# MingXiangL/SPE

Hardware: AMD Instinct MI355X
Metric: images/sec (whole node) at 3x800x1333 bs=2/GPU (higher is better)
Workload: dtype bf16/fp16 operands, fp32 accumulate; 1 GPU; TSCAM_cait_S24 (C=384, depth 24, 8 heads) + 0-layer encoder + 6-layer conditional-DETR decoder x2 stages, 100 queries, COCO heads (91), 2x3x800x1333 per GPU (N=4150 tokens), fwd + SetCriterion + SetCriterionRefine + bwd + grad all-reduce + clip + AdamW; global_batch=2, parallelism=dp1

## Files before the change

### spe_amd/csrc/gemm_bf16tn.hip

```cpp
#include "common.h"

#define GT_BR 64

typedef unsigned int u32x4t_t __attribute__((ext_vector_type(4)));
typedef short s16x4t_t __attribute__((ext_vector_type(4)));
typedef short s16x8t_t __attribute__((ext_vector_type(8)));

struct GemmTNArgs {
    const unsigned short* A; const unsigned short* B; float* C;
    int M, N, R; long lda, ldb, ldc; float alpha;
    int splitk; long slab; int rt_per_split;
};

template <int W>
__device__ __forceinline__ void gt_load(const unsigned short* __restrict__ base, long ld, int r0, int R, int c0, int C, u32x4t_t (&v)[W / 32]) {
    constexpr int CPR = W / 8, RPP = 256 / CPR;
    const int t = threadIdx.x, cc = c0 + (t % CPR) * 8;
    const bool cv = cc < C;
    const int ccl = cv ? cc : 0;
#pragma unroll
    for (int i = 0; i < W / 32; ++i) {
        const int r = r0 + t / CPR + RPP * i;
        const bool ok = cv && r < R;
        const u32x4t_t q = *reinterpret_cast<const u32x4t_t*>(base + (long)min(r, R - 1) * ld + ccl);
        v[i] = ok ? q : (u32x4t_t){0u, 0u, 0u, 0u};
    }
}
template <int W>
__device__ __forceinline__ void gt_stage(unsigned short* lds, const u32x4t_t (&v)[W / 32]) {
    constexpr int CPR = W / 8, RPP = 256 / CPR, LD = W + 8;
    const int t = threadIdx.x;
#pragma unroll
    for (int i = 0; i < W / 32; ++i)
        *reinterpret_cast<u32x4t_t*>(lds + (t / CPR + RPP * i) * LD + (t % CPR) * 8) = v[i];
}
template <int LD>
__device__ __forceinline__ bf16x8_t gt_operand(const unsigned short* tile, int ks, int c0, int lane) {
    typedef __attribute__((address_space(3))) s16x4t_t lds_s4;
    const unsigned short* p = tile + (32 * ks + 8 * (lane >> 4) + ((lane & 15) >> 2)) * LD + c0 + 4 * (lane & 3);
    const s16x4t_t v0 = __builtin_amdgcn_ds_read_tr16_b64_v4i16((lds_s4*)(p));
    const s16x4t_t v1 = __builtin_amdgcn_ds_read_tr16_b64_v4i16((lds_s4*)(p + 4 * LD));
    const s16x8t_t v = __builtin_shufflevector(v0, v1, 0, 1, 2, 3, 4, 5, 6, 7);
    return __builtin_bit_cast(bf16x8_t, v);
}

template <int BM, int BN>
__global__ __launch_bounds__(256) void gemm_bf16tn_kernel(GemmTNArgs p) {
    extern __shared__ __attribute__((aligned(16))) unsigned short smem_tn[];
    constexpr int NFM = BM / 32, NFN = BN / 32, WM = BM / 2, WN = BN / 2;
    constexpr int LDA = BM + 8, LDB = BN + 8;
    constexpr int TA_ = GT_BR * LDA, TB_ = GT_BR * LDB;
    auto sA = [&](int buf) { return smem_tn + buf * (TA_ + TB_); };
    auto sB = [&](int buf) { return smem_tn + buf * (TA_ + TB_) + TA_; };
    const int tiles_m = (p.M + BM - 1) / BM;
    const int tm = blockIdx.x % tiles_m, tn = blockIdx.x / tiles_m;
    const int zs = blockIdx.z;
    float* C = p.C + (long)zs * p.slab;
    const int m0 = tm * BM, n0 = tn * BN;
    const int rtiles = (p.R + GT_BR - 1) / GT_BR;
    const int rt_begin = zs * p.rt_per_split;
    int rt_end = rt_begin + p.rt_per_split; if (rt_end > rtiles) rt_end = rtiles;
    const int nt = rt_end - rt_begin;
    const int lane = threadIdx.x & 63, w = threadIdx.x >> 6;
    const int wm = w >> 1, wn = w & 1, fr = lane & 15;

    f32x4_t acc[NFM][NFN];
#pragma unroll
    for (int i = 0; i < NFM; ++i)
#pragma unroll
        for (int j = 0; j < NFN; ++j) acc[i][j] = (f32x4_t){0.f, 0.f, 0.f, 0.f};

    u32x4t_t ca[BM / 32], cb[BN / 32], na[BM / 32], nb[BN / 32];
#pragma unroll
    for (int i = 0; i < BM / 32; ++i) na[i] = (u32x4t_t){0u, 0u, 0u, 0u};
#pragma unroll
    for (int i = 0; i < BN / 32; ++i) nb[i] = (u32x4t_t){0u, 0u, 0u, 0u};
    if (nt > 0) {
        gt_load<BM>(p.A, p.lda, rt_begin * GT_BR, p.R, m0, p.M, ca);
        gt_load<BN>(p.B, p.ldb, rt_begin * GT_BR, p.R, n0, p.N, cb);
        gt_stage<BM>(sA(0), ca);
        gt_stage<BN>(sB(0), cb);
        if (nt > 1) {
            gt_load<BM>(p.A, p.lda, (rt_begin + 1) * GT_BR, p.R, m0, p.M, ca);
            gt_load<BN>(p.B, p.ldb, (rt_begin + 1) * GT_BR, p.R, n0, p.N, cb);
        }
        __syncthreads();
        for (int t = 0; t < nt; ++t) {
            const int buf = t & 1;
            if (t + 2 < nt) {
                gt_load<BM>(p.A, p.lda, (rt_begin + t + 2) * GT_BR, p.R, m0, p.M, na);
                gt_load<BN>(p.B, p.ldb, (rt_begin + t + 2) * GT_BR, p.R, n0, p.N, nb);
            }
#pragma unroll
            for (int ks = 0; ks < GT_BR / 32; ++ks) {
                bf16x8_t a[NFM], b[NFN];
#pragma unroll
                for (int i = 0; i < NFM; ++i) a[i] = gt_operand<LDA>(sA(buf), ks, wm * WM + i * 16, lane);
#pragma unroll
                for (int j = 0; j < NFN; ++j) b[j] = gt_operand<LDB>(sB(buf), ks, wn * WN + j * 16, lane);
#pragma unroll
                for (int i = 0; i < NFM; ++i)
#pragma unroll
                    for (int j = 0; j < NFN; ++j)
                        acc[i][j] = __builtin_amdgcn_mfma_f32_16x16x32_bf16(b[j], a[i], acc[i][j], 0, 0, 0);
            }
            if (t + 1 < nt) {
                gt_stage<BM>(sA(buf ^ 1), ca);
                gt_stage<BN>(sB(buf ^ 1), cb);
            }
#pragma unroll
            for (int i = 0; i < BM / 32; ++i) ca[i] = na[i];
#pragma unroll
            for (int i = 0; i < BN / 32; ++i) cb[i] = nb[i];
            __syncthreads();
        }
    }
    const bool vst = ((p.ldc & 3) == 0) && ((reinterpret_cast<uintptr_t>(C) & 15) == 0);
#pragma unroll
    for (int j = 0; j < NFN; ++j) {
        const int n = n0 + wn * WN + j * 16 + (lane >> 4) * 4;
        if (n >= p.N) continue;
#pragma unroll
        for (int i = 0; i < NFM; ++i) {
            const int m = m0 + wm * WM + i * 16 + fr;
            if (m >= p.M) continue;
            const long off = (long)m * p.ldc + n;
            float v[4];
#pragma unroll
            for (int r = 0; r < 4; ++r) v[r] = acc[i][j][r] * p.alpha;
            if (vst && n + 3 < p.N) spe_store4_stream(C + off, v[0], v[1], v[2], v[3]);
            else {
#pragma unroll
                for (int r = 0; r < 4; ++r) if (n + r < p.N) C[off + r] = v[r];
            }
        }
    }
}

template <int BM, int BN>
static int launch_tn(const GemmTNArgs& p, hipStream_t stream) {
    constexpr int smem = 2 * GT_BR * ((BM + 8) + (BN + 8)) * (int)sizeof(unsigned short);
    static bool attr_set = false;
    if (!attr_set) {
        hipError_t e = hipFuncSetAttribute(reinterpret_cast<const void*>(&gemm_bf16tn_kernel<BM, BN>),
                                           hipFuncAttributeMaxDynamicSharedMemorySize, smem);
        if (e != hipSuccess) return (int)e;
        attr_set = true;
    }
    const int tiles = ((p.M + BM - 1) / BM) * ((p.N + BN - 1) / BN);
    hipLaunchKernelGGL((gemm_bf16tn_kernel<BM, BN>), dim3(tiles, 1, p.splitk), dim3(256), smem, stream, p);
    SPE_CHECK_LAUNCH();
    return 0;
}

struct TnPlan { int BM, BN, splits, rt_per_split; };
static int tn_gemm_select(int M, int N, int R, long lda, long ldb, int splitk, TnPlan* s) {
    if (M <= 0 || N <= 0) return 1;
    if (R <= 0) return -4;
    if ((lda & 7) || (ldb & 7) || (M & 7) || (N & 7)) return -2;
    const int rtiles = (R + GT_BR - 1) / GT_BR;
    if (splitk < 0) { splitk = -splitk; if (splitk > rtiles) return -5; }
    else if (splitk > 1) return -2;
    if (splitk < 1) splitk = 1;
    s->splits = splitk;
    s->rt_per_split = (rtiles + splitk - 1) / splitk;
    const long t128 = (long)((M + 127) / 128) * ((N + 127) / 128) * splitk;
    static const int small_max = SPE_KNOB("SPE_TN_SMALL_TILES", 256);
    if (t128 < small_max) { s->BM = 64; s->BN = 64; }
    else if (M > 64 && N > 64) { s->BM = 128; s->BN = 128; }
    else if (M > 64) { s->BM = 128; s->BN = 64; }
    else { s->BM = 64; s->BN = 64; }
    return 0;
}

extern "C" int spe_gemm_bf16tn_plan(int M, int N, int R, long lda, long ldb, int splitk, int* v) {
    TnPlan s;
    const int rc = tn_gemm_select(M, N, R, lda, ldb, splitk, &s);
    if (rc < 0) return rc;
    if (rc > 0) s = TnPlan{0, 0, 0, 0};
    if (v) { v[0] = s.BM; v[1] = s.BN; v[2] = s.splits; v[3] = s.rt_per_split; }
    return 0;
}

extern "C" int spe_gemm_bf16tn(const void* A16, const void* B16, float* C, int M, int N, int R, long lda, long ldb, long ldc,
                               float alpha, int splitk, hipStream_t stream) {
    TnPlan s;
    const int rc = tn_gemm_select(M, N, R, lda, ldb, splitk, &s);
    if (rc > 0) return 0;
    if (rc == -4) return rc;
    auto al16 = [](const void* q) { return (reinterpret_cast<uintptr_t>(q) & 15) == 0; };
    if (!al16(A16) || !al16(B16)) return -2;
    if (rc < 0) return rc;
    GemmTNArgs p;
    p.A = reinterpret_cast<const unsigned short*>(A16); p.B = reinterpret_cast<const unsigned short*>(B16); p.C = C;
    p.M = M; p.N = N; p.R = R; p.lda = lda; p.ldb = ldb; p.ldc = ldc; p.alpha = alpha;
    p.slab = splitk < 0 ? (long)M * ldc : 0;
    p.splitk = s.splits;
    p.rt_per_split = s.rt_per_split;
    if (s.BM == 64 && s.BN == 64) return launch_tn<64, 64>(p, stream);
    if (s.BM == 128 && s.BN == 128) return launch_tn<128, 128>(p, stream);
    if (s.BM == 128 && s.BN == 64) return launch_tn<128, 64>(p, stream);
    return -2;
}
```

### spe_amd/csrc/gemm_tiles.h

```cpp
#pragma once

struct TileOrder {
    int xcd_bind;
    int grid;
};

static inline TileOrder tile_order(int M, int N, int tiles_m, int tiles_n) {
    TileOrder o{0, tiles_m * tiles_n};
    if (M >= N && tiles_m >= 16) o.xcd_bind = 1;
    else if (N > M && tiles_n >= 16) o.xcd_bind = 2;
    else if (tiles_m >= 16) o.xcd_bind = 1;
    else if (tiles_n >= 16) o.xcd_bind = 2;
    if (o.xcd_bind == 1) o.grid = 8 * ((tiles_m + 7) / 8) * tiles_n;
    if (o.xcd_bind == 2) o.grid = 8 * ((tiles_n + 7) / 8) * tiles_m;
    return o;
}

__device__ __forceinline__ bool tile_decode(int xcd_bind, int tiles_m, int tiles_n, int& tm, int& tn) {
    if (xcd_bind == 0) { tm = blockIdx.x % tiles_m; tn = blockIdx.x / tiles_m; }
    else {
        const int no = (xcd_bind == 1) ? tiles_n : tiles_m;
        const int xcd = blockIdx.x & 7, idx = blockIdx.x >> 3;
        const int tb = xcd + 8 * (idx / no), to = idx % no;
        tm = (xcd_bind == 1) ? tb : to; tn = (xcd_bind == 1) ? to : tb;
        if (tm >= tiles_m || tn >= tiles_n) return false;
    }
    return true;
}

__device__ __forceinline__ void glds16(const void* gsrc, unsigned lds_dst) {
    unsigned keep;
    asm volatile("s_mov_b32 %0, m0\n\ts_mov_b32 m0, %2\n\ts_nop 0\n\tglobal_load_lds_dwordx4 %1, off\n\ts_mov_b32 m0, %0"
                 : "=&s"(keep) : "v"(gsrc), "s"(lds_dst) : "memory");
}
```

Baseline: 41.84 images/sec.

## Remap TN GEMM blocks to XCD-contiguous chunks and unroll 64x64 double-buffer ping-pong

```diff
diff --git a/spe_amd/csrc/gemm_bf16tn.hip b/spe_amd/csrc/gemm_bf16tn.hip
--- a/spe_amd/csrc/gemm_bf16tn.hip
+++ b/spe_amd/csrc/gemm_bf16tn.hip
@@ -1,4 +1,5 @@
 #include "common.h"
+#include "gemm_tiles.h"
 
 #define GT_BR 64
 
@@ -16,23 +17,23 @@
 __device__ __forceinline__ void gt_load(const unsigned short* __restrict__ base, long ld, int r0, int R, int c0, int C, u32x4t_t (&v)[W / 32]) {
     constexpr int CPR = W / 8, RPP = 256 / CPR;
     const int t = threadIdx.x, cc = c0 + (t % CPR) * 8;
-    const bool cv = cc < C;
-    const int ccl = cv ? cc : 0;
+    const int ccl = cc < C ? cc : 0;
 #pragma unroll
     for (int i = 0; i < W / 32; ++i) {
         const int r = r0 + t / CPR + RPP * i;
-        const bool ok = cv && r < R;
-        const u32x4t_t q = *reinterpret_cast<const u32x4t_t*>(base + (long)min(r, R - 1) * ld + ccl);
-        v[i] = ok ? q : (u32x4t_t){0u, 0u, 0u, 0u};
+        v[i] = *reinterpret_cast<const u32x4t_t*>(base + (long)min(r, R - 1) * ld + ccl);
     }
 }
 template <int W>
-__device__ __forceinline__ void gt_stage(unsigned short* lds, const u32x4t_t (&v)[W / 32]) {
+__device__ __forceinline__ void gt_stage(unsigned short* lds, const u32x4t_t (&v)[W / 32], int r0, int R, int c0, int C) {
     constexpr int CPR = W / 8, RPP = 256 / CPR, LD = W + 8;
     const int t = threadIdx.x;
-#pragma unroll
-    for (int i = 0; i < W / 32; ++i)
-        *reinterpret_cast<u32x4t_t*>(lds + (t / CPR + RPP * i) * LD + (t % CPR) * 8) = v[i];
+    const bool cv = c0 + (t % CPR) * 8 < C;
+#pragma unroll
+    for (int i = 0; i < W / 32; ++i) {
+        const unsigned keep = (cv && r0 + t / CPR + RPP * i < R) ? ~0u : 0u;
+        *reinterpret_cast<u32x4t_t*>(lds + (t / CPR + RPP * i) * LD + (t % CPR) * 8) = v[i] & (u32x4t_t){keep, keep, keep, keep};
+    }
 }
 template <int LD>
 __device__ __forceinline__ bf16x8_t gt_operand(const unsigned short* tile, int ks, int c0, int lane) {
@@ -52,9 +53,10 @@
     constexpr int TA_ = GT_BR * LDA, TB_ = GT_BR * LDB;
     auto sA = [&](int buf) { return smem_tn + buf * (TA_ + TB_); };
     auto sB = [&](int buf) { return smem_tn + buf * (TA_ + TB_) + TA_; };
-    const int tiles_m = (p.M + BM - 1) / BM;
-    const int tm = blockIdx.x % tiles_m, tn = blockIdx.x / tiles_m;
-    const int zs = blockIdx.z;
+    const int tiles_m = (p.M + BM - 1) / BM, tiles_n = (p.N + BN - 1) / BN;
+    int tile, zs;
+    if (!tn_decode(blockIdx.x, tiles_m * tiles_n, p.splitk, tile, zs)) return;
+    const int tm = tile % tiles_m, tn = tile / tiles_m;
     float* C = p.C + (long)zs * p.slab;
     const int m0 = tm * BM, n0 = tn * BN;
     const int rtiles = (p.R + GT_BR - 1) / GT_BR;
@@ -75,22 +77,20 @@
     for (int i = 0; i < BM / 32; ++i) na[i] = (u32x4t_t){0u, 0u, 0u, 0u};
 #pragma unroll
     for (int i = 0; i < BN / 32; ++i) nb[i] = (u32x4t_t){0u, 0u, 0u, 0u};
+    auto load_tile = [&](int t, u32x4t_t (&xa)[BM / 32], u32x4t_t (&xb)[BN / 32]) {
+        gt_load<BM>(p.A, p.lda, (rt_begin + t) * GT_BR, p.R, m0, p.M, xa);
+        gt_load<BN>(p.B, p.ldb, (rt_begin + t) * GT_BR, p.R, n0, p.N, xb);
+    };
+    auto stage_tile = [&](int buf, int t, const u32x4t_t (&ya)[BM / 32], const u32x4t_t (&yb)[BN / 32]) {
+        gt_stage<BM>(sA(buf), ya, (rt_begin + t) * GT_BR, p.R, m0, p.M);
+        gt_stage<BN>(sB(buf), yb, (rt_begin + t) * GT_BR, p.R, n0, p.N);
+    };
     if (nt > 0) {
-        gt_load<BM>(p.A, p.lda, rt_begin * GT_BR, p.R, m0, p.M, ca);
-        gt_load<BN>(p.B, p.ldb, rt_begin * GT_BR, p.R, n0, p.N, cb);
-        gt_stage<BM>(sA(0), ca);
-        gt_stage<BN>(sB(0), cb);
-        if (nt > 1) {
-            gt_load<BM>(p.A, p.lda, (rt_begin + 1) * GT_BR, p.R, m0, p.M, ca);
-            gt_load<BN>(p.B, p.ldb, (rt_begin + 1) * GT_BR, p.R, n0, p.N, cb);
-        }
+        load_tile(0, ca, cb);
+        stage_tile(0, 0, ca, cb);
+        if (nt > 1) load_tile(1, ca, cb);
         __syncthreads();
-        for (int t = 0; t < nt; ++t) {
-            const int buf = t & 1;
-            if (t + 2 < nt) {
-                gt_load<BM>(p.A, p.lda, (rt_begin + t + 2) * GT_BR, p.R, m0, p.M, na);
-                gt_load<BN>(p.B, p.ldb, (rt_begin + t + 2) * GT_BR, p.R, n0, p.N, nb);
-            }
+        auto multiply = [&](int buf) {
 #pragma unroll
             for (int ks = 0; ks < GT_BR / 32; ++ks) {
                 bf16x8_t a[NFM], b[NFN];
@@ -104,15 +104,34 @@
                     for (int j = 0; j < NFN; ++j)
                         acc[i][j] = __builtin_amdgcn_mfma_f32_16x16x32_bf16(b[j], a[i], acc[i][j], 0, 0, 0);
             }
-            if (t + 1 < nt) {
-                gt_stage<BM>(sA(buf ^ 1), ca);
-                gt_stage<BN>(sB(buf ^ 1), cb);
+        };
+        if constexpr (BM == 64 && BN == 64) {
+            auto step = [&](int t, u32x4t_t (&ya)[BM / 32], u32x4t_t (&yb)[BN / 32], u32x4t_t (&xa)[BM / 32], u32x4t_t (&xb)[BN / 32]) {
+                load_tile(t + 2, xa, xb);
+                multiply(t & 1);
+                stage_tile((t & 1) ^ 1, t + 1, ya, yb);
+                __syncthreads();
+            };
+            auto last = [&](int t, u32x4t_t (&ya)[BM / 32], u32x4t_t (&yb)[BN / 32]) {
+                multiply(t & 1);
+                if (t + 1 < nt) stage_tile((t & 1) ^ 1, t + 1, ya, yb);
+                __syncthreads();
+            };
+            int t = 0;
+            for (; t + 3 < nt; t += 2) { step(t, ca, cb, na, nb); step(t + 1, na, nb, ca, cb); }
+            if (t + 2 < nt) { step(t, ca, cb, na, nb); last(t + 1, na, nb); last(t + 2, na, nb); }
+            else { last(t, ca, cb); if (t + 1 < nt) last(t + 1, ca, cb); }
+        } else {
+            for (int t = 0; t < nt; ++t) {
+                if (t + 2 < nt) load_tile(t + 2, na, nb);
+                multiply(t & 1);
+                if (t + 1 < nt) stage_tile((t & 1) ^ 1, t + 1, ca, cb);
+#pragma unroll
+                for (int i = 0; i < BM / 32; ++i) ca[i] = na[i];
+#pragma unroll
+                for (int i = 0; i < BN / 32; ++i) cb[i] = nb[i];
+                __syncthreads();
             }
-#pragma unroll
-            for (int i = 0; i < BM / 32; ++i) ca[i] = na[i];
-#pragma unroll
-            for (int i = 0; i < BN / 32; ++i) cb[i] = nb[i];
-            __syncthreads();
         }
     }
     const bool vst = ((p.ldc & 3) == 0) && ((reinterpret_cast<uintptr_t>(C) & 15) == 0);
@@ -148,7 +167,7 @@
         attr_set = true;
     }
     const int tiles = ((p.M + BM - 1) / BM) * ((p.N + BN - 1) / BN);
-    hipLaunchKernelGGL((gemm_bf16tn_kernel<BM, BN>), dim3(tiles, 1, p.splitk), dim3(256), smem, stream, p);
+    hipLaunchKernelGGL((gemm_bf16tn_kernel<BM, BN>), dim3(tn_order(tiles, p.splitk).grid), dim3(256), smem, stream, p);
     SPE_CHECK_LAUNCH();
     return 0;
 }
diff --git a/spe_amd/csrc/gemm_tiles.h b/spe_amd/csrc/gemm_tiles.h
--- a/spe_amd/csrc/gemm_tiles.h
+++ b/spe_amd/csrc/gemm_tiles.h
@@ -1,4 +1,29 @@
 #pragma once
+
+#if defined(__HIP__) || defined(__HIPCC__)
+#define GT_HOST_DEVICE __host__ __device__ __forceinline__
+#else
+#define GT_HOST_DEVICE inline
+#endif
+
+struct TnOrder {
+    int per;
+    int grid;
+};
+
+static inline TnOrder tn_order(int tiles, int splits) {
+    const int per = (tiles * splits + 7) / 8;
+    return TnOrder{per, 8 * per};
+}
+
+GT_HOST_DEVICE bool tn_decode(int b, int tiles, int splits, int& tile, int& split) {
+    const int total = tiles * splits, q = total >> 3, r = total & 7;
+    const int x = b & 7, i = b >> 3;
+    if (i >= q + (x < r ? 1 : 0)) return false;
+    const int linear = x * q + (x < r ? x : r) + i;
+    split = linear / tiles; tile = linear - split * tiles;
+    return true;
+}
 
 struct TileOrder {
     int xcd_bind;
@@ -16,6 +41,7 @@
     return o;
 }
 
+#if defined(__HIP__) || defined(__HIPCC__)
 __device__ __forceinline__ bool tile_decode(int xcd_bind, int tiles_m, int tiles_n, int& tm, int& tn) {
     if (xcd_bind == 0) { tm = blockIdx.x % tiles_m; tn = blockIdx.x / tiles_m; }
     else {
@@ -33,3 +59,4 @@
     asm volatile("s_mov_b32 %0, m0\n\ts_mov_b32 m0, %2\n\ts_nop 0\n\tglobal_load_lds_dwordx4 %1, off\n\ts_mov_b32 m0, %0"
                  : "=&s"(keep) : "v"(gsrc), "s"(lds_dst) : "memory");
 }
+#endif
```

New measurement: 41.88 images/sec (median of 2 runs). No clear change (+0.1%).
